# thu-nics/MixDQ

Hardware: AMD Instinct MI355X
Metric: sdxl_turbo_unet_w8a8_images_per_sec (higher is better)
Workload: dtype int8; 1 GPU; sdxl_turbo_unet_w8a8_1024px_bs1_1step; global_batch=1, per_gpu_batch=1, px=1024, latent=128, unet_forwards_per_image=1, unet_rows_per_image=1, graphs_cached=1, w_config=weight/uniform_8, a_config=act/act_8.00, bos=True, parallelism=dp1 (batch-sharded replicas, no step-loop collective), hip_graph=True, producer_fusions=True, swap_glue=False, w4_kernel_layers=0, quantizable_layers=794

## Files before the change

### __graft_entry__.py

```python
import os
import sys

ROOT = os.path.dirname(os.path.abspath(__file__))
if ROOT not in sys.path:
    sys.path.insert(0, ROOT)


def build() -> None:
    from mixdq_amd.build import build as build_hip
    lib = build_hip(force=False, verbose=True)
    assert os.path.exists(lib)
    from oracle import oracle as O
    O.build()
    import mixdq_amd._C as C
    import mixdq_amd.nn
    import mixdq_amd.quantize_sdxl
    import mixdq_amd.unet
    import mixdq_amd.text
    import mixdq_amd.image
    assert C.ABI_VERSION == 3
    print("build ok:", lib)


def smoke() -> None:
# ... 143 lines not shown
    xs, es = dd.f32(80, (2051,), -9, 9), dd.normal_f16(81, (2, 2056), 1.0)
    nz = dd.f32(82, (4, 2052), -2, 2)
    xs_d, in_d = t(xs), torch.zeros((2, 2056), dtype=torch.float16, device=dev)
    step_d, t_d = torch.tensor([1], dtype=torch.int32, device=dev), scal(-1.0)
    C.sampler_step(xs_d, t(es), in_d, t(sch.coef), t(sch.t_table), step_d, t_d, 7.5, 2, t(nz), n=2051, row_stride=2056,
                   noise_stride=2052)
    xs_ref, in_ref = sampler_ref.step(xs, es[0, :2051], es[1, :2051], sch.coef[1], 7.5, nz[1, :2051])
    assert np.array_equal(xs_d.cpu().numpy().view(np.uint32), xs_ref.view(np.uint32)), "sampler state mismatch"
    for r in range(2):
        assert np.array_equal(in_d[r, :2051].cpu().numpy().view(np.uint16), in_ref.view(np.uint16)), "sampler input"
    assert int(step_d.item()) == 2 and float(t_d.item()) == float(sch.timesteps[2]), "sampler step state"
    from tests import inpaint9_ref
    rng = np.random.default_rng(9)
    img = rng.integers(0, 256, (1, 3, 16, 24), dtype=np.uint8)
    msk = np.where(rng.random((1, 16, 24)) < 0.05, 255, 0).astype(np.uint8)
    grown = C.mask_dilate(t(msk), 2)
    assert np.array_equal(grown.cpu().numpy(), inpaint9_ref.mask_dilate(msk, 2)), "mask_dilate mismatch"
    blank = C.image_to_nhwc8_f16(t(img), grown).permute(0, 2, 3, 1).contiguous().cpu().numpy()
    assert np.array_equal(blank.view(np.uint16), inpaint9_ref.ingest_masked(img, grown.cpu().numpy()).view(np.uint16)), \
        "blanked ingest mismatch"
    ml, zl = dd.f32(90, (1, 2, 3), 0, 1), dd.f32(91, (1, 2, 3, 4), -3, 3)
    cnd = C.inpaint_cond(t(ml), t(zl).permute(0, 3, 1, 2)).permute(0, 2, 3, 1).contiguous().cpu().numpy()
    assert np.array_equal(cnd.view(np.uint16), inpaint9_ref.inpaint_cond(ml, zl).view(np.uint16)), "inpaint_cond mismatch"
    torch.cuda.synchronize()
    print("smoke ok: sampler step and the inpainting launches bit-exact vs their restatements; quantize, qlinear, qconv2d, qlinear_geglu, grouped GEMM, GroupNorm bit-exact vs oracle; "
          "fused cross-attention == its two-launch chain; the persistent GEMM + GEGLU kernel and a swapped "
          "GroupNorm + SiLU module bit-exact; attention and FP16 layers within tolerance "
          "on", torch.cuda.get_device_name(0))


if __name__ == "__main__":
    build()
    if "--smoke" in sys.argv:
        smoke()
```

### include/mixdq_hip.h

```cpp
#ifndef MIXDQ_HIP_H_
#define MIXDQ_HIP_H_

#include <stddef.h>
#include <stdint.h>

#ifdef __cplusplus
extern "C" {
#endif

#define MIXDQ_ABI_VERSION 3

typedef void* mixdq_stream_t;

enum mixdq_status {
  MIXDQ_OK = 0,
  MIXDQ_ERR_INVALID_ARG = 1,
  MIXDQ_ERR_ALIGNMENT = 2,
  MIXDQ_ERR_UNSUPPORTED = 3,
  MIXDQ_ERR_LAUNCH = 4,
  MIXDQ_ERR_W4_SHAPE = 5,
  MIXDQ_ERR_GEGLU_SHAPE = 6,
  MIXDQ_ERR_PADDING = 7,
  MIXDQ_ERR_ROWMAP_RESIDUAL = 8,
  MIXDQ_ERR_SHAPE = 9,
// ... 135 lines not shown
                         const float* scale_inv, const float* zero_point,
                         int8_t* out_q_or_null, void* out_f16_or_null, int flags,
                         mixdq_stream_t stream);

int mixdq_qlinear_w8a8_attn(const int8_t* A, const int8_t* W, const float* bias0, const float* scale,
                            const void* k_f16, const void* v_f16, void* out, int64_t M, int N, int K,
                            int rows_per_image, int tkv, int64_t k_batch_stride, int k_row_stride,
                            int64_t v_batch_stride, int v_row_stride, float softmax_scale,
                            const float* out_scale_inv_or_null, const float* out_zero_point_or_null,
                            int flags, mixdq_stream_t stream);

typedef struct mixdq_gemm_group {
  const int8_t* W;
  const float* bias0;
  const float* scale;
  const void* bias_f16_or_null;
  void* D_f16;
  int32_t N;
  int32_t reserved;
} mixdq_gemm_group;
int mixdq_qlinear_w8a8_grouped(const int8_t* A, const mixdq_gemm_group* groups_device, int ngroups,
                               int64_t M, int max_N, int K, int group_rows, int group_stride,
                               int group_offset, int flags, mixdq_stream_t stream);

int mixdq_qlinear_w8a8_geglu(const int8_t* A, const int8_t* W_interleaved, const float* bias0,
                             const float* scale, const void* bias_f16_or_null, int8_t* out_i8,
                             int64_t M, int N, int K, const float* out_scale_inv,
                             const float* out_zero_point, int flags, mixdq_stream_t stream);

int mixdq_attention_f16(const void* q_f16, const void* k_f16, const void* v_f16, void* out,
                        int batch, int heads, int head_dim, int tq, int tkv,
                        int64_t q_batch_stride, int64_t q_row_stride,
                        int64_t k_batch_stride, int64_t k_row_stride,
                        int64_t v_batch_stride, int64_t v_row_stride,
                        int64_t out_batch_stride, int64_t out_row_stride,
                        float softmax_scale, const float* out_scale_inv_or_null,
                        const float* out_zero_point_or_null, int flags, mixdq_stream_t stream);

int mixdq_attention_f16_prefetch(const void* q_f16, const void* k_f16, const void* v_f16, void* out,
                                 int batch, int heads, int head_dim, int tq, int tkv,
                                 int64_t q_batch_stride, int64_t q_row_stride,
                                 int64_t k_batch_stride, int64_t k_row_stride,
                                 int64_t v_batch_stride, int64_t v_row_stride,
                                 int64_t out_batch_stride, int64_t out_row_stride,
                                 float softmax_scale, const float* out_scale_inv_or_null,
                                 const float* out_zero_point_or_null,
// ... 119 lines not shown
```

### mixdq_amd/_C.py

```python
from __future__ import annotations

import ctypes
import os

import torch

_PKG = os.path.dirname(os.path.abspath(__file__))
LIB_PATH = os.environ.get("MIXDQ_HIP_LIB") or os.path.join(_PKG, "libmixdq_hip.so")

if not os.path.exists(LIB_PATH):
    raise ImportError(
        f"{LIB_PATH} not found: the HIP extension has not been built. Run "
        "`python -m mixdq_amd.build` (needs hipcc). There is no CPU fallback.")

_lib = ctypes.CDLL(LIB_PATH)

_vp, _i64, _i32, _sz = ctypes.c_void_p, ctypes.c_int64, ctypes.c_int, ctypes.c_size_t
_lib.mixdq_status_string.restype = ctypes.c_char_p
_lib.mixdq_status_string.argtypes = [_i32]
_lib.mixdq_abi_version.restype = _i32
_lib.mixdq_quantize_f16_i8.argtypes = [_vp, _vp, _vp, _vp, _vp, _i32, _vp, _vp, _i32, _vp]
_lib.mixdq_qlinear_w8a8.argtypes = [_vp, _vp, _vp, _vp, _vp, _vp, _i64, _i32, _i32, _i32, _vp]
_lib.mixdq_qlinear_w8a8_rows.argtypes = [_vp, _vp, _vp, _vp, _vp, _vp, _i64, _i32, _i32,
                                         _i32, _i32, _i32, _vp, _i64, _i32, _vp]
# ... 493 lines not shown
        _check(all(m[0].size(1) == self.members[0][0].size(1) for m in self.members),
               "members of a grouped launch share K")
        self.max_N = max(r[5] for r in rows)
        self.n = len(rows)
        self.table = torch.from_numpy(np.asarray(rows, dtype=np.int64)).to(self.members[0][0].device)
        self.key = tuple(r[0] for r in rows) + tuple(r[4] for r in rows)


def qlinear_grouped(input_int8, table: "GemmGroupTable", *, _row_map=None, _cfg=0):
    _check(input_int8.is_cuda and input_int8.dtype == torch.int8, "input_int8 should be int8 on GPU")
    _check(input_int8.size(-1) == table.K, "The last dimension of input and weight should match")
    a = input_int8.contiguous()
    M = a.numel() // table.K if table.K else 0
    rm = _row_map or (0, 0, 0)
    _record("linear_grouped", M, sum(m[0].size(0) for m in table.members), table.K, table.K,
            table.w4, qlinear_grouped,
            (input_int8, table), dict(_row_map=_row_map, _cfg=_cfg), w2=table.w2)
    with torch.cuda.device(a.device):
        code = _lib.mixdq_qlinear_w8a8_grouped(a.data_ptr(), table.table.data_ptr(), table.n, M,
                                               table.max_N, table.K, rm[0], rm[1], rm[2],
                                               FLAGS | (_cfg << 8) | _wflag(table.w4, table.w2),
                                               _stream())
    _status(code, "qlinear_grouped")


_lib.mixdq_qlinear_w8a8_attn.argtypes = [_vp] * 7 + [_i64, _i32, _i32, _i32, _i32, _i64, _i32, _i64,
                                          _i32, ctypes.c_float, _vp, _vp, _i32, _vp]
_lib.mixdq_qlinear_w8a8_attn.restype = _i32


def qlinear_attention_supported(x_shape, N, K, k) -> bool:
    return (len(x_shape) == 3 and N % 128 == 0 and K % 128 == 0 and x_shape[1] % 64 == 0
            and k.dim() == 3 and 0 < k.shape[1] <= 128 and k.shape[2] == N
            and x_shape[0] * x_shape[1] * K < 2 ** 32 and N * K < 2 ** 32)


def qlinear_attention(input_int8, weight_int8, scale, bias0, k, v, scale_inv=None, zero_point=None,
                      softmax_scale=None, *, _w4=False, _w2=False, _abits=8):
    _trace_w(weight_int8)
    _check(input_int8.is_cuda and input_int8.dtype == torch.int8 and input_int8.dim() == 3,
           "input_int8 should be an int8 [B, T, K] GPU tensor")
    _check(weight_int8.dtype == torch.int8, "weight_int8 should be int8 type")
    wflag = _wflag(_w4, _w2)
    N, K = weight_int8.size(0), weight_int8.size(1) * _kmul(_w4, _w2)
    B, T, _ = input_int8.shape
    _check(input_int8.size(-1) == K, "The last dimension of input and weight should match")
# ... 1005 lines not shown
```

### mixdq_amd/build.py

```python
import os
import subprocess
import sys

PKG = os.path.dirname(os.path.abspath(__file__))
CSRC = os.path.join(PKG, "csrc")
LIB = os.path.join(PKG, "libmixdq_hip.so")
SOURCES = ["quantize.hip", "igemm.hip", "igemm_aq.hip", "igemm_ln.hip", "iconv.hip", "fused_norm.hip", "attention.hip",
           "sampler.hip", "vae.hip", "image.hip"]
HEADERS = ["common.h", "attn_core.h", "iconv.h", "igemm_kernel.h", "igemm_pp.h", "f16in_table.h", os.path.join("..", "..", "include", "mixdq_hip.h"),
           os.path.join("..", "..", "include", "mixdq_math.h")]
FLAGS = ["--offload-arch=gfx950", "-O3", "-std=c++17", "-fPIC", "-ffp-contract=off",
         "-fno-fast-math", "-Wall", "-Wno-unused-function"]
EXTRA = {"attention.hip": ["-mllvm", "-amdgpu-mfma-vgpr-form=1"],
         "igemm.hip": ["-mllvm", "-amdgpu-kernarg-preload-count=14"],
         "igemm_aq.hip": ["-mllvm", "-amdgpu-kernarg-preload-count=14"],
         "igemm_ln.hip": ["-mllvm", "-amdgpu-kernarg-preload-count=14"]}
OBJ = os.path.join(PKG, "_obj")


def _hipcc():
    for c in (os.environ.get("HIPCC"), "/opt/rocm/bin/hipcc", "hipcc"):
        if c and (os.path.sep not in c or os.path.exists(c)):
            return c
    return "hipcc"


def csrc_sha16() -> str:
    import hashlib
    h = hashlib.sha256()
    for name in sorted(os.listdir(CSRC)):
        if name.endswith((".hip", ".h")):
            with open(os.path.join(CSRC, name), "rb") as f:
                h.update(name.encode() + b"\0" + f.read())
    return h.hexdigest()[:16]


def _build_info_obj(force: bool) -> str:
    src = os.path.join(OBJ, "build_info.cpp")
    obj = os.path.join(OBJ, "build_info.o")
    text = ('extern "C" __attribute__((visibility("default"))) const char* mixdq_build_csrc_sha16() '
            '{ return "%s"; }\n' % csrc_sha16())
    if force or not os.path.exists(src) or open(src).read() != text or not os.path.exists(obj):
        with open(src, "w") as f:
            f.write(text)
        subprocess.check_call(["g++", "-O1", "-fPIC", "-c", "-o", obj, src])
    return obj


def _aq_asm_cmd(asm: str):
    src = os.path.join(CSRC, "igemm_aq.hip")
    return [_hipcc()] + FLAGS + EXTRA.get("igemm_aq.hip", []) + ["--cuda-device-only", "-S", "-o", asm, src]


def _check_aq_isa(asm: str, obj: str) -> None:
    tool = os.path.join(os.path.dirname(PKG), "tools", "check_aq_isa.py")
    if not os.path.exists(tool):
# ... 53 lines not shown
```

### mixdq_amd/unet.py

```python
from __future__ import annotations

import math
import weakref
from collections import OrderedDict

import torch
import torch.nn as nn
import torch.nn.functional as F

DEFUSE = False


class defused:

    def __enter__(self):
        global DEFUSE
        self.saved, DEFUSE = DEFUSE, True

    def __exit__(self, *exc):
        global DEFUSE
        DEFUSE = self.saved


def _accel(m) -> bool:
# ... 286 lines not shown
    projection_class_embeddings_input_dim=None,
    use_linear_projection=False,
    norm_num_groups=32,
)

SDXL_INPAINT_CONFIG = dict(SDXL_CONFIG, in_channels=9)
SD15_INPAINT_CONFIG = dict(SD15_CONFIG, in_channels=9)


def head_width(cfg, channels: int) -> int:
    heads = cfg.get("num_attention_heads")
    if heads:
        if channels % heads:
            raise ValueError(f"{channels} channels do not split into {heads} heads")
        return channels // heads
    return cfg["head_dim"]


def _linear_proj(cfg) -> bool:
    return bool(cfg.get("use_linear_projection", True))


def sinusoidal_embedding(t: torch.Tensor, dim: int) -> torch.Tensor:
    half = dim // 2
    key = (half, t.device)
    freqs = _SIN_FREQS.get(key)
    if freqs is None:
        exponent = -math.log(10000.0) * torch.arange(half, dtype=torch.float32, device=t.device) / half
        freqs = torch.exp(exponent)
        if not (t.is_cuda and torch.cuda.is_current_stream_capturing()):
            _SIN_FREQS[key] = freqs
    emb = t.float()[:, None] * freqs[None, :]
    return torch.cat([torch.cos(emb), torch.sin(emb)], dim=-1)


_SIN_FREQS = {}


class TimestepEmbedding(nn.Module):
    def __init__(self, in_dim, dim):
        super().__init__()
        self.linear_1 = nn.Linear(in_dim, dim)
        self.linear_2 = nn.Linear(dim, dim)

    def forward(self, x):
        return self.linear_2(F.silu(self.linear_1(x)))


class ResnetBlock2D(nn.Module):
    def __init__(self, cin, cout, temb_dim, groups, split=0):
        super().__init__()
        self.norm1 = nn.GroupNorm(groups, cin, eps=1e-5)
        self.conv1 = nn.Conv2d(cin, cout, 3, 1, 1)
        self.time_emb_proj = nn.Linear(temb_dim, cout)
        self.norm2 = nn.GroupNorm(groups, cout, eps=1e-5)
        self.conv2 = nn.Conv2d(cout, cout, 3, 1, 1)
        self.conv_shortcut = nn.Conv2d(cin, cout, 1, 1, 0) if cin != cout else None
        self.nonlinearity = nn.SiLU()
        if self.conv_shortcut is not None and split:
# ... 646 lines not shown
            table = self._grouped("kv", (g, K, wb, B, T), [
                (pk["w"], pk["bias0"], pk["scale"], None, o) for _, pk, o in members], wb)
            _C.qlinear_grouped(x_int, table, _row_map=(T - 1, T, 1))

    @staticmethod
    def _kv_pack(blk, context=None):
        lk, lv = blk.attn2.to_k, blk.attn2.to_v
        layers = [lk, lv]
        if not (all(getattr(m, "valid_for_acceleration", False) and getattr(m, "bos", False)
                    and m.bias is None for m in layers)
                and lk.out_features == lv.out_features):
            return None
        if context is not None and not (context.dtype == torch.float16 and context.shape[1] > 1):
            return None
        if len(set(_quantizer_groups(_memo(blk), "kv", layers))) != 1:
            return None
        if not _uniform_storage(layers):
            return None
        pack = blk.__dict__.get("_kvpack")
        if not _pack_valid(pack, layers):
            pack = blk.__dict__["_kvpack"] = _pack_rows(layers)
        return pack

    def _project_temb_ahead(self, emb):
        resnets = [m for m in self.modules() if isinstance(m, ResnetBlock2D)]
        if not resnets or not emb.is_cuda:
            return
        s = F.silu(emb)
        B = s.shape[0]
        acc = [r.time_emb_proj for r in resnets if _accel(r.time_emb_proj)]
        ok = _fusable_f16(s) and s.dim() == 2
        gid = dict(zip(map(id, acc), _quantizer_groups(_memo(self), "temb", acc)))
        shared, grouped = {}, {}
        for res in resnets:
            layer = res.time_emb_proj
            if not (_accel(layer) and ok):
                res._t = (layer(s), None)
                continue
            bufs = layer.__dict__.setdefault("_t_out", {})
            buf = bufs.get((B, s.device))
            if buf is None:
                buf = bufs[(B, s.device)] = torch.empty((B, layer.out_features),
                                                        dtype=torch.float16, device=s.device)
            res._t = (buf, None)
            grouped.setdefault((gid[id(layer)], layer.in_features, _wbits(layer)),
                               []).append((layer, buf))
        from mixdq_amd import _C
        for (g, K, wb), members in grouped.items():
            if g not in shared:
                shared[g] = members[0][0]._quant(s)
            x_int = shared[g]
            if len(members) == 1:
                members[0][0]._gemm(x_int, out=members[0][1])
                continue
            table = self._grouped("temb", (g, K, wb, B), [
                (m.weight_storage()[0], m.bias0, m.scale, m.bias, buf)
                for m, buf in members], wb)
            _C.qlinear_grouped(x_int, table)

    def refresh_derived_(self):
        with torch.no_grad():
            for m in self.modules():
                if m is not self and hasattr(m, "refresh_derived_"):
                    m.refresh_derived_()
                bufs = m.__dict__.get("_kv_buf")
                if bufs and torch.is_tensor(getattr(m, "bos_pre_computed", None)):
                    for slot in bufs.values():
                        slot[1][:, :1, :] = m.bos_pre_computed.to(slot[1].device)
                        slot[0] = None
                pack = m.__dict__.get("_kvpack")
                if pack is not None and pack.get("outs"):
                    lk, lv = (r() for r in pack["layers"])
                    if lk is None or lv is None:
                        continue
                    for slot in pack["outs"].values():
                        slot[1][:, :1, :] = torch.cat(
                            [lk.bos_pre_computed, lv.bos_pre_computed], dim=-1).to(slot[1].device)
                        slot[0] = None
        return self

    def prepare_fused_(self):
# ... 110 lines not shown
                raise RuntimeError(f"SDXLUNet.forward: this UNet has {cc} conditioning channels: a {co}-channel sample "
                                   f"needs cond_term= (unet.cond_term(cond)), or pass all {co + cc} channels")
            return
        if cc <= 0:
            raise RuntimeError("SDXLUNet.forward: cond_term given, but this UNet has no conditioning channels")
        if sample.dim() != 4 or sample.shape[1] != co:
            raise RuntimeError(f"SDXLUNet.forward: with cond_term the sample should have {co} channels")
        want = (sample.shape[0], self.conv_in.out_channels, sample.shape[2], sample.shape[3])
        if not (torch.is_tensor(cond_term) and tuple(cond_term.shape) == want and cond_term.dtype == sample.dtype
                and cond_term.device == sample.device
                and cond_term.is_contiguous(memory_format=torch.channels_last)):
            raise RuntimeError(f"SDXLUNet.forward: cond_term should be a channels-last {sample.dtype} tensor of shape "
                               f"{want} (one row per sample row) on the sample's device")

    def forward(self, sample, timestep, encoder_hidden_states, added_cond_kwargs=None,
                return_dict=False, cond_term=None):
        cfg = self.cfg
        self._check_cond_term(sample, cond_term)
        B = sample.shape[0]
        dtype = sample.dtype
        t = timestep
        if not torch.is_tensor(t):
            t = torch.tensor([t], dtype=torch.float32, device=sample.device)
        t = t.reshape(-1).expand(B)
        emb = self.time_embedding(sinusoidal_embedding(t, cfg["block_out_channels"][0]).to(dtype))
        if cfg.get("addition_embed_type", "text_time") is not None:
            time_ids = added_cond_kwargs["time_ids"]
            text_embeds = added_cond_kwargs["text_embeds"]
            tid = sinusoidal_embedding(time_ids.flatten(), cfg["addition_time_embed_dim"])
            add = torch.cat([text_embeds, tid.reshape(B, -1).to(dtype)], dim=-1)
            emb = emb + self.add_embedding(add)

        use_pf = bool(self.fused and PREFETCH and sample.is_cuda and _fusable_f16(sample) and not DEFUSE)
        if not use_pf:
            return self._forward_body(sample, emb, encoder_hidden_states, cond_term)
        from mixdq_amd import _C
        plans = self.__dict__.setdefault("_pf_plans", {})
        plan = plans.get(sample.device)
        if plan is not None and not _plan_alive(plan, sample.device):
            plans.pop(sample.device, None)
            plan = None
        ctx = _C.PrefetchContext(sample.device, plan["lists"] if plan else None)
        try:
            with ctx:
                return self._forward_body(sample, emb, encoder_hidden_states, cond_term)
        finally:
            if ctx._outer is None:
                sig = _trace_signature(ctx.trace)
                if plan is None or plan["sig"] != sig:
                    new = _build_prefetch_plan(ctx.trace)
                    if new is None:
                        plans.pop(sample.device, None)
                    else:
                        plans[sample.device] = new

    def _apply(self, fn, recurse=True):
        self.__dict__.pop("_pf_plans", None)
        self.__dict__.pop("_cin_split", None)
        return super()._apply(fn, recurse)

    def load_state_dict(self, *args, **kwargs):
        self.__dict__.pop("_pf_plans", None)
        return super().load_state_dict(*args, **kwargs)

    def _forward_body(self, sample, emb, encoder_hidden_states, cond_term=None):
        if self.fused and _fusable_f16(sample) and not DEFUSE:
            self._project_temb_ahead(emb)
            self._project_context_ahead(encoder_hidden_states)
        x = sample.contiguous(memory_format=torch.channels_last)
        x = self.conv_in(x) if cond_term is None else self._conv_in_with_term(x, cond_term)
        skips = [x]
        for blk in self.down_blocks:
            x, outs = blk(x, emb, encoder_hidden_states)
            skips += outs
        x = self.mid_block(x, emb, encoder_hidden_states)
        for blk in self.up_blocks:
            x = blk(x, skips, emb, encoder_hidden_states)
        if self.fused and _fusable_f16(x):
            feed, q = _gn_feed(self.conv_norm_out, x, self.conv_out, silu=True)
            x = self.conv_out.forward_quantized(feed) if q else self.conv_out(feed)
        else:
            x = self.conv_out(self.conv_act(self.conv_norm_out(x)))
        return (x,)


def quantizable_layers(unet: nn.Module) -> "OrderedDict[str, nn.Module]":
    return OrderedDict((n, m) for n, m in unet.named_modules()
                       if isinstance(m, (nn.Linear, nn.Conv2d)))


# ... 19 lines not shown
```

Baseline: 92.19 images/s.

## Fuse conditioning embeddings into a cond prologue with grouped GEMV kernels

Adds a cond_embed kernel that builds the sinusoidal timestep and time-id embeddings and quantizes them directly. It also adds a grouped int8 GEMV kernel with SiLU+quantize and pair-add epilogues that computes the time/add embedding MLPs and writes the quantized temb inputs for the resnets. Together these replace the many small torch ops and GEMM launches at the start of the UNet forward. The path runs by default when batch is small, at the cost of a second code path and extra buffers.

Result: no change. 92.80 images/s (median of 6 runs) (+0.7%).

```diff
diff --git a/__graft_entry__.py b/__graft_entry__.py
--- a/__graft_entry__.py
+++ b/__graft_entry__.py
@@ -189,6 +189,16 @@
     ml, zl = dd.f32(90, (1, 2, 3), 0, 1), dd.f32(91, (1, 2, 3, 4), -3, 3)
     cnd = C.inpaint_cond(t(ml), t(zl).permute(0, 3, 1, 2)).permute(0, 2, 3, 1).contiguous().cpu().numpy()
     assert np.array_equal(cnd.view(np.uint16), inpaint9_ref.inpaint_cond(ml, zl).view(np.uint16)), "inpaint_cond mismatch"
+    gm, gw = [], []
+    for i, (n_out, k_in) in enumerate(((128, 320), (64, 192))):
+        xi, wi = dd.int8(95 + i, (2, k_in)), dd.int8(97 + i, (n_out, k_in))
+        b0i, sci = dd.f32(99 + i, (n_out,), -200, 200), dd.f32(101 + i, (n_out,), 2e-4, 9e-4)
+        oi = torch.zeros((2, n_out), dtype=torch.float16, device=dev)
+        gm.append((t(xi), t(wi), t(b0i), t(sci), None, oi, None, None, None))
+        gw.append(O.qlinear(xi, wi, b0i, sci, None, variant))
+    C.qlinear_gemv_grouped(C.GemvTable(gm))
+    for m_, want in zip(gm, gw):
+        assert np.array_equal(m_[5].cpu().numpy().view(np.uint16), want.view(np.uint16)), "GEMV mismatch"
     torch.cuda.synchronize()
     print("smoke ok: sampler step and the inpainting launches bit-exact vs their restatements; quantize, qlinear, qconv2d, qlinear_geglu, grouped GEMM, GroupNorm bit-exact vs oracle; "
           "fused cross-attention == its two-launch chain; the persistent GEMM + GEGLU kernel and a swapped "
diff --git a/include/mixdq_hip.h b/include/mixdq_hip.h
--- a/include/mixdq_hip.h
+++ b/include/mixdq_hip.h
@@ -181,6 +181,39 @@
 int mixdq_qlinear_w8a8_grouped(const int8_t* A, const mixdq_gemm_group* groups_device, int ngroups,
                                int64_t M, int max_N, int K, int group_rows, int group_stride,
                                int group_offset, int flags, mixdq_stream_t stream);
+
+typedef struct mixdq_gemv_group {
+  const int8_t* W;
+  const float* bias0;
+  const float* scale;
+  const void* bias_f16_or_null;
+  void* D_f16_or_null;
+  int32_t N;
+  int32_t K;
+  const int8_t* A;
+  int8_t* Q_or_null;
+  const float* q_scale_inv;
+  const float* q_zero_point;
+} mixdq_gemv_group;
+typedef struct mixdq_quant_out {
+  int8_t* out;
+  const float* scale_inv;
+  const float* zero_point;
+} mixdq_quant_out;
+enum { MIXDQ_GEMV_PLAIN = 0, MIXDQ_GEMV_SILU_QUANT = 1, MIXDQ_GEMV_PAIR_ADD_SILU_QUANT = 2 };
+#define MIXDQ_GEMV_MAX_PAIR_OUTS 8
+int mixdq_qlinear_w8a8_gemv_grouped(const mixdq_gemv_group* groups_device, const mixdq_gemv_group* groups_host,
+                                    int ngroups, int64_t M, int epilogue, const mixdq_quant_out* pair_outs,
+                                    int n_pair_outs, void* emb_f16_or_null, void* silu_f16_or_null, int flags,
+                                    mixdq_stream_t stream);
+int mixdq_qlinear_gemv_max_rows(void);
+
+enum { MIXDQ_COND_F32 = 0, MIXDQ_COND_F16 = 1, MIXDQ_COND_I64 = 2, MIXDQ_COND_I32 = 3, MIXDQ_COND_F64 = 4 };
+int mixdq_cond_embed(const void* timestep, int t_dtype, int t_count, const void* time_ids, int ids_dtype, int n_ids,
+                     const void* text_f16, int64_t text_row_stride, int P, const float* freqs0, int half0,
+                     const float* freqs1, int half1, void* out0, const float* scale_inv0, const float* zero_point0,
+                     void* out1, const float* scale_inv1, const float* zero_point1, int B, int flags,
+                     mixdq_stream_t stream);
 
 int mixdq_qlinear_w8a8_geglu(const int8_t* A, const int8_t* W_interleaved, const float* bias0,
                              const float* scale, const void* bias_f16_or_null, int8_t* out_i8,
diff --git a/mixdq_amd/_C.py b/mixdq_amd/_C.py
--- a/mixdq_amd/_C.py
+++ b/mixdq_amd/_C.py
@@ -539,6 +539,129 @@
                                                FLAGS | (_cfg << 8) | _wflag(table.w4, table.w2),
                                                _stream())
     _status(code, "qlinear_grouped")
+
+
+if not hasattr(_lib, "mixdq_qlinear_w8a8_gemv_grouped"):
+    raise ImportError(f"{LIB_PATH} does not export mixdq_qlinear_w8a8_gemv_grouped (rebuild with "
+                      "`python -m mixdq_amd.build --force`)")
+_lib.mixdq_qlinear_w8a8_gemv_grouped.argtypes = [_vp, _vp, _i32, _i64, _i32, _vp, _i32, _vp, _vp, _i32, _vp]
+_lib.mixdq_qlinear_w8a8_gemv_grouped.restype = _i32
+_lib.mixdq_qlinear_gemv_max_rows.argtypes = []
+_lib.mixdq_qlinear_gemv_max_rows.restype = _i32
+_lib.mixdq_cond_embed.argtypes = [_vp, _i32, _i32, _vp, _i32, _i32, _vp, _i64, _i32, _vp, _i32, _vp, _i32,
+                                  _vp, _vp, _vp, _vp, _vp, _vp, _i32, _i32, _vp]
+_lib.mixdq_cond_embed.restype = _i32
+
+GEMV_MAX_ROWS = int(_lib.mixdq_qlinear_gemv_max_rows())
+GEMV_MAX_PAIR_OUTS = 8
+GEMV_EPILOGUES = {None: 0, "silu_quant": 1, "pair": 2}
+COND_DTYPES = {torch.float32: 0, torch.float16: 1, torch.int64: 2, torch.int32: 3, torch.float64: 4}
+
+
+def cond_prologue_enabled() -> bool:
+    return os.environ.get("MIXDQ_COND_PROLOGUE", "1") != "0"
+
+
+def gemv_wanted(M: int) -> bool:
+    return 0 < int(M) <= GEMV_MAX_ROWS
+
+
+class GemvTable:
+
+    def __init__(self, members):
+        import numpy as np
+        rows, keep = [], []
+        self.M = None
+        for a, w, b0, sc, bias, out, q_out, q_sinv, q_zp in members:
+            _check(w.is_cuda and w.dtype == torch.int8 and w.dim() == 2 and w.is_contiguous(), "member weight: int8 [N, K]")
+            N, K = w.shape
+            _check(a.is_cuda and a.dtype == torch.int8 and a.is_contiguous() and a.dim() >= 1 and a.shape[-1] == K,
+                   "member input: contiguous int8 [..., K]")
+            M = a.numel() // K if K else 0
+            _check(self.M in (None, M), "members of a GEMV launch have the same number of rows")
+            self.M = M
+            b0, sc = _f32vec(b0), _f32vec(sc)
+            bias = None if bias is None else bias.contiguous()
+            _check(b0.numel() == N and sc.numel() == N and (bias is None or (bias.numel() == N and bias.dtype == torch.float16)),
+                   "member epilogue vectors should have N elements (bias: fp16)")
+            for t, dt, n in ((out, torch.float16, "out"), (q_out, torch.int8, "q_out")):
+                _check(t is None or (t.is_cuda and t.dtype == dt and t.is_contiguous() and t.numel() == M * N),
+                       f"member {n}: contiguous [M, N]")
+            _check((q_out is None) == (q_sinv is None) == (q_zp is None), "q_out comes with its quantizer")
+            _check(q_sinv is None or (q_sinv.dtype == torch.float32 and q_zp.dtype == torch.float32),
+                   "quantizer parameters should be fp32")
+            keep.append((a, w, b0, sc, bias, out, q_out, q_sinv, q_zp))
+            rows.append([w.data_ptr(), b0.data_ptr(), sc.data_ptr(), _ptr(bias) or 0, _ptr(out) or 0,
+                         int(N) | (int(K) << 32), a.data_ptr(), _ptr(q_out) or 0, _ptr(q_sinv) or 0, _ptr(q_zp) or 0])
+        self._keep = keep
+        self.n = len(rows)
+        self.shapes = tuple((r[5] & 0xffffffff, r[5] >> 32) for r in rows)
+        self.host = np.ascontiguousarray(np.asarray(rows, dtype=np.int64).reshape(self.n, 10))
+        self.table = torch.from_numpy(self.host).to(keep[0][0].device) if rows else None
+        self.key = tuple(v for r in rows for v in r)
+
+
+def qlinear_gemv_grouped(table: "GemvTable", *, _epilogue=None, _pair_outs=(), _emb=None, _silu=None):
+    import numpy as np
+    _check(_epilogue in GEMV_EPILOGUES, f"_epilogue: one of {list(GEMV_EPILOGUES)}")
+    if table.n == 0 or not table.M:
+        return
+    dev = table.table.device
+    po = None
+    if _epilogue == "pair":
+        _check(len(_pair_outs) <= GEMV_MAX_PAIR_OUTS, f"at most {GEMV_MAX_PAIR_OUTS} pair outputs")
+        N = table.shapes[0][0]
+        for q, s, z in _pair_outs:
+            _check(q.is_cuda and q.dtype == torch.int8 and q.is_contiguous() and q.numel() == table.M * N
+                   and s.dtype == torch.float32 and z.dtype == torch.float32 and s.device == dev and z.device == dev,
+                   "pair output: contiguous int8 [M, N] with fp32 quantizer parameters")
+        for t in (_emb, _silu):
+            _check(t is None or (t.is_cuda and t.dtype == torch.float16 and t.is_contiguous()
+                                 and t.numel() == table.M * N), "emb / silu: contiguous fp16 [M, N]")
+        po = np.ascontiguousarray(np.asarray([[q.data_ptr(), s.data_ptr(), z.data_ptr()] for q, s, z in _pair_outs],
+                                             dtype=np.int64).reshape(len(_pair_outs), 3))
+    else:
+        _check(not _pair_outs and _emb is None and _silu is None, "pair outputs belong to the pair epilogue")
+    _record("linear_gemv", table.M, sum(s[0] for s in table.shapes), max(s[1] for s in table.shapes),
+            min(s[1] for s in table.shapes), False, qlinear_gemv_grouped, (table,),
+            dict(_epilogue=_epilogue, _pair_outs=_pair_outs, _emb=_emb, _silu=_silu))
+    with torch.cuda.device(dev):
+        code = _lib.mixdq_qlinear_w8a8_gemv_grouped(
+            table.table.data_ptr(), table.host.ctypes.data, table.n, table.M, GEMV_EPILOGUES[_epilogue],
+            None if po is None or not len(po) else po.ctypes.data, 0 if po is None else len(po), _ptr(_emb), _ptr(_silu),
+            FLAGS, _stream())
+    _status(code, "qlinear_gemv_grouped")
+
+
+def cond_embed(timestep, time_ids, text_embeds, freqs0, freqs1, q0=None, q1=None, *, _out0=None, _out1=None):
+    dev = text_embeds.device
+    _check(text_embeds.is_cuda and text_embeds.dtype == torch.float16 and text_embeds.dim() == 2
+           and (text_embeds.shape[1] == 0 or text_embeds.stride(1) == 1), "text_embeds should be fp16 [B, P] on GPU")
+    B, P = text_embeds.shape
+    _check(timestep.device == dev and timestep.dtype in COND_DTYPES and timestep.numel() in (1, B)
+           and timestep.is_contiguous(), "timestep: 1 or B values on the device")
+    _check(time_ids.device == dev and time_ids.dtype in COND_DTYPES and time_ids.dim() == 2 and time_ids.shape[0] == B
+           and time_ids.is_contiguous(), "time_ids: contiguous [B, n] on the device")
+    for f in (freqs0, freqs1):
+        _check(f.device == dev and f.dtype == torch.float32 and f.dim() == 1 and f.is_contiguous(), "freqs: fp32 vector")
+    for q in (q0, q1):
+        _check(q is None or all(t.device == dev and t.dtype == torch.float32 for t in q), "quantizer parameters: fp32")
+    h0, h1, n = freqs0.numel(), freqs1.numel(), time_ids.shape[1]
+    outs = []
+    for given, q, width in ((_out0, q0, 2 * h0), (_out1, q1, P + n * 2 * h1)):
+        dt = torch.float16 if q is None else torch.int8
+        _check(given is None or (given.device == dev and given.dtype == dt and given.shape == (B, width)
+                                 and given.is_contiguous()), "_out<i>: a contiguous [B, width] buffer of the output's type")
+        outs.append(torch.empty((B, width), dtype=dt, device=dev) if given is None else given)
+    out0, out1 = outs
+    with torch.cuda.device(dev):
+        code = _lib.mixdq_cond_embed(
+            timestep.data_ptr(), COND_DTYPES[timestep.dtype], timestep.numel(), time_ids.data_ptr(),
+            COND_DTYPES[time_ids.dtype], n, text_embeds.data_ptr(), text_embeds.stride(0) if B > 1 else P, P,
+            freqs0.data_ptr(), h0, freqs1.data_ptr(), h1, out0.data_ptr(), _ptr(q0 and q0[0]), _ptr(q0 and q0[1]),
+            out1.data_ptr(), _ptr(q1 and q1[0]), _ptr(q1 and q1[1]), B, FLAGS, _stream())
+    _status(code, "cond_embed")
+    return out0, out1
 
 
 _lib.mixdq_qlinear_w8a8_attn.argtypes = [_vp] * 7 + [_i64, _i32, _i32, _i32, _i32, _i64, _i32, _i64,
diff --git a/mixdq_amd/build.py b/mixdq_amd/build.py
--- a/mixdq_amd/build.py
+++ b/mixdq_amd/build.py
@@ -4,9 +4,10 @@
 
 PKG = os.path.dirname(os.path.abspath(__file__))
 CSRC = os.path.join(PKG, "csrc")
+INCLUDE = os.path.join(os.path.dirname(PKG), "include")
 LIB = os.path.join(PKG, "libmixdq_hip.so")
 SOURCES = ["quantize.hip", "igemm.hip", "igemm_aq.hip", "igemm_ln.hip", "iconv.hip", "fused_norm.hip", "attention.hip",
-           "sampler.hip", "vae.hip", "image.hip"]
+           "sampler.hip", "vae.hip", "image.hip", "cond.hip"]
 HEADERS = ["common.h", "attn_core.h", "iconv.h", "igemm_kernel.h", "igemm_pp.h", "f16in_table.h", os.path.join("..", "..", "include", "mixdq_hip.h"),
            os.path.join("..", "..", "include", "mixdq_math.h")]
 FLAGS = ["--offload-arch=gfx950", "-O3", "-std=c++17", "-fPIC", "-ffp-contract=off",
@@ -32,6 +33,10 @@
         if name.endswith((".hip", ".h")):
             with open(os.path.join(CSRC, name), "rb") as f:
                 h.update(name.encode() + b"\0" + f.read())
+    for name in sorted(os.listdir(INCLUDE)):
+        if name.endswith(".h"):
+            with open(os.path.join(INCLUDE, name), "rb") as f:
+                h.update(b"include/" + name.encode() + b"\0" + f.read())
     return h.hexdigest()[:16]
 
 
diff --git a/mixdq_amd/csrc/cond.hip b/mixdq_amd/csrc/cond.hip
--- /dev/null
+++ b/mixdq_amd/csrc/cond.hip
@@ -0,0 +1,340 @@
+#include "common.h"
+
+namespace mixdq {
+namespace {
+
+__device__ __forceinline__ float load_as_float(const void* p, int dtype, int64_t i) {
+  switch (dtype) {
+    case MIXDQ_COND_F16: return __half2float(reinterpret_cast<const __half*>(p)[i]);
+    case MIXDQ_COND_I64: return (float)reinterpret_cast<const int64_t*>(p)[i];
+    case MIXDQ_COND_I32: return (float)reinterpret_cast<const int32_t*>(p)[i];
+    case MIXDQ_COND_F64: return (float)reinterpret_cast<const double*>(p)[i];
+    default: return reinterpret_cast<const float*>(p)[i];
+  }
+}
+
+__device__ __forceinline__ __half silu_f16(__half h) {
+  const float x = __half2float(h);
+  const float e = expf(-x);
+  return f32_to_f16_rn(x / __fadd_rn(1.0f, e));
+}
+
+__device__ __forceinline__ int8_t quantize_f16(__half h, float s_inv, float zp, bool unfused) {
+  const float x = __half2float(h);
+  return (int8_t)(unfused ? quantize_one<true>(x, s_inv, zp) : quantize_one<false>(x, s_inv, zp));
+}
+
+struct EmbedArgs {
+  const void* t; const void* ids; const __half* text;
+  const float* f0; const float* f1;
+  void* out0; void* out1;
+  const float* s0; const float* z0; const float* s1; const float* z1;
+  int64_t text_stride;
+  int t_dtype, t_n, ids_dtype, n_ids, P, half0, half1, B, unfused;
+};
+
+__global__ __launch_bounds__(256) void cond_embed_kernel(EmbedArgs a) {
+  const int w0 = 2 * a.half0, w1 = a.P + a.n_ids * 2 * a.half1;
+  const int64_t e = (int64_t)blockIdx.x * blockDim.x + threadIdx.x;
+  if (e >= (int64_t)a.B * (w0 + w1)) return;
+  const int b = (int)(e / (w0 + w1));
+  int c = (int)(e - (int64_t)b * (w0 + w1));
+  const bool second = c >= w0;
+  __half h;
+  if (second && c - w0 < a.P) {
+    c -= w0;
+    h = a.text[b * a.text_stride + c];
+  } else {
+    float v;
+    const float* f;
+    int half, i;
+    if (!second) {
+      v = load_as_float(a.t, a.t_dtype, a.t_n > 1 ? b : 0);
+      f = a.f0; half = a.half0; i = c;
+    } else {
+      c -= w0;
+      const int r = c - a.P;
+      v = load_as_float(a.ids, a.ids_dtype, (int64_t)b * a.n_ids + r / (2 * a.half1));
+      f = a.f1; half = a.half1; i = r % (2 * a.half1);
+    }
+    const bool is_sin = i >= half;
+    const float arg = __fmul_rn(v, f[is_sin ? i - half : i]);
+    h = f32_to_f16_rn(is_sin ? sinf(arg) : cosf(arg));
+  }
+  void* out = second ? a.out1 : a.out0;
+  const float* sp = second ? a.s1 : a.s0;
+  const float* zp = second ? a.z1 : a.z0;
+  const int64_t o = (int64_t)b * (second ? w1 : w0) + c;
+  if (sp) reinterpret_cast<int8_t*>(out)[o] = quantize_f16(h, *sp, *zp, a.unfused != 0);
+  else reinterpret_cast<__half*>(out)[o] = h;
+}
+
+constexpr int kGemvMaxRows = 8;
+constexpr int kGemvWaves = 4;
+constexpr int kGemvTargetWaves = 4096;
+constexpr int kGemvMaxLds = 64 * 1024;
+
+__host__ __device__ inline int gemv_lanes(int K) {
+  const int chunks = K >> 4;
+  int l = 4;
+  while (l < 64 && l * 4 < chunks) l <<= 1;
+  return l;
+}
+
+struct PairOuts {
+  mixdq_quant_out q[MIXDQ_GEMV_MAX_PAIR_OUTS];
+  int n;
+  __half* emb; __half* silu;
+};
+
+template <int MR>
+__device__ __forceinline__ void gemv_dot(const mixdq_gemv_group& g, const char* a_lds, int col, bool valid, int kl,
+                                         int lanes, int (&acc)[MR]) {
+  const int chunks = g.K >> 4;
+  const uint4* wrow = reinterpret_cast<const uint4*>(g.W + (int64_t)col * g.K);
+#pragma unroll
+  for (int m = 0; m < MR; ++m) acc[m] = 0;
+  for (int j0 = kl; j0 < chunks; j0 += 4 * lanes) {
+    uint4 w[4];
+#pragma unroll
+    for (int u = 0; u < 4; ++u) {
+      const int j = j0 + u * lanes;
+      w[u] = (valid && j < chunks) ? wrow[j] : make_uint4(0, 0, 0, 0);
+    }
+#pragma unroll
+    for (int u = 0; u < 4; ++u) {
+      const int j = min(j0 + u * lanes, chunks - 1);
+#pragma unroll
+      for (int m = 0; m < MR; ++m) {
+        const uint4 av = *reinterpret_cast<const uint4*>(a_lds + m * g.K + j * 16);
+        int s = acc[m];
+        s = __builtin_amdgcn_sdot4((int)av.x, (int)w[u].x, s, false);
+        s = __builtin_amdgcn_sdot4((int)av.y, (int)w[u].y, s, false);
+        s = __builtin_amdgcn_sdot4((int)av.z, (int)w[u].z, s, false);
+        s = __builtin_amdgcn_sdot4((int)av.w, (int)w[u].w, s, false);
+        acc[m] = s;
+      }
+    }
+  }
+}
+
+template <int MR, int EPI>
+__global__ __launch_bounds__(256) void gemv_kernel(const mixdq_gemv_group* __restrict__ groups, int M, int ppt,
+                                                   int unfused_, PairOuts po) {
+  extern __shared__ __attribute__((aligned(16))) char gemv_lds[];
+  constexpr int NM = EPI == 2 ? 2 : 1;
+  mixdq_gemv_group g[NM];
+#pragma unroll
+  for (int h = 0; h < NM; ++h) g[h] = groups[blockIdx.y * NM + h];
+  const int N = g[0].N;
+  int lanes = gemv_lanes(g[0].K);
+  if (NM == 2) lanes = max(lanes, gemv_lanes(g[NM - 1].K));
+  const int cpp = 64 / lanes;
+  const int cw = ppt * cpp;
+  const int block_col0 = blockIdx.x * (kGemvWaves * cw);
+  if (block_col0 >= N) return;
+  const bool unfused = unfused_ != 0;
+
+  int a_off[NM];
+  {
+    int off = 0;
+#pragma unroll
+    for (int h = 0; h < NM; ++h) {
+      a_off[h] = off;
+      const int chunks = g[h].K >> 4;
+      const uint4* src = reinterpret_cast<const uint4*>(g[h].A);
+      uint4* dst = reinterpret_cast<uint4*>(gemv_lds + off);
+      for (int i = threadIdx.x; i < MR * chunks; i += blockDim.x)
+        dst[i] = i < M * chunks ? src[i] : make_uint4(0, 0, 0, 0);
+      off += MR * g[h].K;
+    }
+  }
+  float q_sinv = 0.f, q_zp = 0.f;
+  if constexpr (EPI == 1) { q_sinv = *g[0].q_scale_inv; q_zp = *g[0].q_zero_point; }
+  float p_sinv[MIXDQ_GEMV_MAX_PAIR_OUTS], p_zp[MIXDQ_GEMV_MAX_PAIR_OUTS];
+  if constexpr (EPI == 2) {
+#pragma unroll
+    for (int i = 0; i < MIXDQ_GEMV_MAX_PAIR_OUTS; ++i)
+      if (i < po.n) { p_sinv[i] = *po.q[i].scale_inv; p_zp[i] = *po.q[i].zero_point; }
+  }
+  __syncthreads();
+
+  const int lane = threadIdx.x & 63, wave = threadIdx.x >> 6;
+  const int kl = lane & (lanes - 1), sub = lane / lanes;
+  const int wave_col0 = block_col0 + wave * cw;
+  for (int p = 0; p < ppt; ++p) {
+    const int c0 = wave_col0 + p * cpp;
+    if (c0 >= N) break;
+    const int col = c0 + sub;
+    const bool valid = col < N;
+    const int colc = valid ? col : N - 1;
+    float b0[NM], sc[NM], bs[NM];
+#pragma unroll
+    for (int h = 0; h < NM; ++h) {
+      b0[h] = g[h].bias0[colc];
+      sc[h] = g[h].scale[colc];
+      bs[h] = g[h].bias_f16_or_null ? __half2float(reinterpret_cast<const __half*>(g[h].bias_f16_or_null)[colc]) : 0.f;
+    }
+    int acc[NM][MR];
+#pragma unroll
+    for (int h = 0; h < NM; ++h) gemv_dot<MR>(g[h], gemv_lds + a_off[h], colc, valid, kl, lanes, acc[h]);
+#pragma unroll
+    for (int o = 32; o >= 1; o >>= 1) {
+      if (o < lanes) {
+#pragma unroll
+        for (int h = 0; h < NM; ++h)
+#pragma unroll
+          for (int m = 0; m < MR; ++m) acc[h][m] += __shfl_xor(acc[h][m], o);
+      }
+    }
+#pragma unroll
+    for (int m = 0; m < MR; ++m) {
+      if (kl != 0 || !valid || m >= M) break;
+      const int64_t o = (int64_t)m * N + col;
+      __half d[NM];
+#pragma unroll
+      for (int h = 0; h < NM; ++h) {
+        d[h] = epilogue_one(acc[h][m], b0[h], sc[h], bs[h], g[h].bias_f16_or_null != nullptr, unfused);
+        if (g[h].D_f16_or_null) reinterpret_cast<__half*>(g[h].D_f16_or_null)[o] = d[h];
+      }
+      if constexpr (EPI == 1) {
+        g[0].Q_or_null[o] = quantize_f16(silu_f16(d[0]), q_sinv, q_zp, unfused);
+      } else if constexpr (EPI == 2) {
+        const __half emb = f32_to_f16_rn(__fadd_rn(__half2float(d[0]), __half2float(d[NM - 1])));
+        const __half s = silu_f16(emb);
+        if (po.emb) po.emb[o] = emb;
+        if (po.silu) po.silu[o] = s;
+#pragma unroll
+        for (int i = 0; i < MIXDQ_GEMV_MAX_PAIR_OUTS; ++i)
+          if (i < po.n) po.q[i].out[o] = quantize_f16(s, p_sinv[i], p_zp[i], unfused);
+      }
+    }
+  }
+}
+
+template <int EPI>
+int launch_gemv(const mixdq_gemv_group* dev, int M, int ppt, int unfused, const PairOuts& po, dim3 grid, int lds,
+                hipStream_t stream) {
+#define GEMV_GO(MR) gemv_kernel<MR, EPI><<<grid, 64 * kGemvWaves, lds, stream>>>(dev, M, ppt, unfused, po)
+  if (M == 1) GEMV_GO(1);
+  else if (M == 2) GEMV_GO(2);
+  else if (M <= 4) GEMV_GO(4);
+  else GEMV_GO(8);
+#undef GEMV_GO
+  return launch_status();
+}
+
+inline bool dtype_ok(int d) { return d >= MIXDQ_COND_F32 && d <= MIXDQ_COND_F64; }
+inline int dtype_size(int d) { return d == MIXDQ_COND_F16 ? 2 : (d == MIXDQ_COND_F32 || d == MIXDQ_COND_I32) ? 4 : 8; }
+
+}
+}
+
+using namespace mixdq;
+
+extern "C" int mixdq_qlinear_gemv_max_rows(void) { return kGemvMaxRows; }
+
+extern "C" int mixdq_cond_embed(const void* timestep, int t_dtype, int t_count, const void* time_ids, int ids_dtype,
+                                int n_ids, const void* text_f16, int64_t text_row_stride, int P, const float* freqs0,
+                                int half0, const float* freqs1, int half1, void* out0, const float* scale_inv0,
+                                const float* zero_point0, void* out1, const float* scale_inv1,
+                                const float* zero_point1, int B, int flags, mixdq_stream_t stream) {
+  if (flags & ~MIXDQ_FLAG_UNFUSED) return MIXDQ_ERR_UNSUPPORTED;
+  if (B < 0 || P < 0 || n_ids < 0 || half0 < 0 || half1 < 0 || text_row_stride < 0) return MIXDQ_ERR_INVALID_ARG;
+  if (!dtype_ok(t_dtype) || !dtype_ok(ids_dtype) || (t_count != 1 && t_count != B)) return MIXDQ_ERR_INVALID_ARG;
+  if ((scale_inv0 == nullptr) != (zero_point0 == nullptr) || (scale_inv1 == nullptr) != (zero_point1 == nullptr))
+    return MIXDQ_ERR_INVALID_ARG;
+  const int64_t w0 = 2 * (int64_t)half0, w1 = (int64_t)P + (int64_t)n_ids * 2 * half1;
+  if (w0 + w1 > INT32_MAX) return MIXDQ_ERR_SHAPE;
+  const int64_t total = (int64_t)B * (w0 + w1);
+  if (total == 0) return MIXDQ_OK;
+  if ((w0 && (!timestep || !freqs0 || !out0)) || (w1 && !out1) || (P && !text_f16) ||
+      (n_ids * half1 && (!time_ids || !freqs1)))
+    return MIXDQ_ERR_INVALID_ARG;
+  if (((uintptr_t)timestep % dtype_size(t_dtype)) || ((uintptr_t)time_ids % dtype_size(ids_dtype)) ||
+      ((uintptr_t)text_f16 & 1) || (((uintptr_t)freqs0 | (uintptr_t)freqs1) & 3) ||
+      (!scale_inv0 && ((uintptr_t)out0 & 1)) || (!scale_inv1 && ((uintptr_t)out1 & 1)))
+    return MIXDQ_ERR_ALIGNMENT;
+  EmbedArgs a;
+  a.t = timestep; a.ids = time_ids; a.text = (const __half*)text_f16;
+  a.f0 = freqs0; a.f1 = freqs1; a.out0 = out0; a.out1 = out1;
+  a.s0 = scale_inv0; a.z0 = zero_point0; a.s1 = scale_inv1; a.z1 = zero_point1;
+  a.text_stride = text_row_stride;
+  a.t_dtype = t_dtype; a.t_n = t_count; a.ids_dtype = ids_dtype; a.n_ids = n_ids; a.P = P;
+  a.half0 = half0; a.half1 = half1; a.B = B; a.unfused = (flags & MIXDQ_FLAG_UNFUSED) ? 1 : 0;
+  const int64_t blocks = (total + 255) / 256;
+  if (blocks > INT32_MAX) return MIXDQ_ERR_SHAPE;
+  cond_embed_kernel<<<(int)blocks, 256, 0, (hipStream_t)stream>>>(a);
+  return launch_status();
+}
+
+extern "C" int mixdq_qlinear_w8a8_gemv_grouped(const mixdq_gemv_group* groups_device,
+                                               const mixdq_gemv_group* groups_host, int ngroups, int64_t M,
+                                               int epilogue, const mixdq_quant_out* pair_outs, int n_pair_outs,
+                                               void* emb_f16_or_null, void* silu_f16_or_null, int flags,
+                                               mixdq_stream_t stream) {
+  if (flags & ~MIXDQ_FLAG_UNFUSED) return MIXDQ_ERR_UNSUPPORTED;
+  if (M < 0 || ngroups < 0 || n_pair_outs < 0) return MIXDQ_ERR_INVALID_ARG;
+  if (epilogue < MIXDQ_GEMV_PLAIN || epilogue > MIXDQ_GEMV_PAIR_ADD_SILU_QUANT) return MIXDQ_ERR_INVALID_ARG;
+  if (M == 0 || ngroups == 0) return MIXDQ_OK;
+  if (M > kGemvMaxRows) return MIXDQ_ERR_SHAPE;
+  if (!groups_device || !groups_host || ngroups > 65535) return MIXDQ_ERR_INVALID_ARG;
+  const bool pair = epilogue == MIXDQ_GEMV_PAIR_ADD_SILU_QUANT;
+  const int nm = pair ? 2 : 1;
+  PairOuts po{};
+  if (pair) {
+    if (ngroups != 2 || n_pair_outs > MIXDQ_GEMV_MAX_PAIR_OUTS || (n_pair_outs && !pair_outs))
+      return MIXDQ_ERR_INVALID_ARG;
+    if (groups_host[0].N != groups_host[1].N) return MIXDQ_ERR_SHAPE;
+    for (int i = 0; i < n_pair_outs; ++i) {
+      if (!pair_outs[i].out || !pair_outs[i].scale_inv || !pair_outs[i].zero_point) return MIXDQ_ERR_INVALID_ARG;
+      po.q[i] = pair_outs[i];
+    }
+    po.n = n_pair_outs;
+    po.emb = (__half*)emb_f16_or_null;
+    po.silu = (__half*)silu_f16_or_null;
+    if (((uintptr_t)po.emb | (uintptr_t)po.silu) & 1) return MIXDQ_ERR_ALIGNMENT;
+  } else if (n_pair_outs || emb_f16_or_null || silu_f16_or_null) {
+    return MIXDQ_ERR_INVALID_ARG;
+  }
+  const int mr = M == 1 ? 1 : M == 2 ? 2 : M <= 4 ? 4 : 8;
+  int64_t passes = 0;
+  int lds = 0;
+  for (int i = 0; i < ngroups; i += nm) {
+    int lanes = 0, lds_i = 0;
+    for (int h = 0; h < nm; ++h) {
+      const mixdq_gemv_group& g = groups_host[i + h];
+      if (!g.W || !g.bias0 || !g.scale || !g.A || g.N <= 0 || g.K <= 0) return MIXDQ_ERR_INVALID_ARG;
+      if (g.N % 4 != 0 || g.K % 16 != 0 || (((uintptr_t)g.W | (uintptr_t)g.A) & 15) ||
+          (((uintptr_t)g.bias0 | (uintptr_t)g.scale) & 3) ||
+          (((uintptr_t)g.bias_f16_or_null | (uintptr_t)g.D_f16_or_null) & 1))
+        return MIXDQ_ERR_ALIGNMENT;
+      if (epilogue == MIXDQ_GEMV_SILU_QUANT && (!g.Q_or_null || !g.q_scale_inv || !g.q_zero_point))
+        return MIXDQ_ERR_INVALID_ARG;
+      if (epilogue == MIXDQ_GEMV_PLAIN && !g.D_f16_or_null) return MIXDQ_ERR_INVALID_ARG;
+      lanes = lanes > gemv_lanes(g.K) ? lanes : gemv_lanes(g.K);
+      lds_i += mr * g.K;
+    }
+    if (lds_i > kGemvMaxLds) return MIXDQ_ERR_SHAPE;
+    lds = lds > lds_i ? lds : lds_i;
+    const int cpp = 64 / lanes;
+    passes += (groups_host[i].N + cpp - 1) / cpp;
+  }
+  int64_t ppt = passes / kGemvTargetWaves;
+  if (ppt < 1) ppt = 1;
+  if (ppt > 1024) ppt = 1024;
+  int gx = 1;
+  for (int i = 0; i < ngroups; i += nm) {
+    int lanes = 0;
+    for (int h = 0; h < nm; ++h) lanes = lanes > gemv_lanes(groups_host[i + h].K) ? lanes : gemv_lanes(groups_host[i + h].K);
+    const int64_t cols_per_block = (int64_t)kGemvWaves * ppt * (64 / lanes);
+    const int64_t bx = (groups_host[i].N + cols_per_block - 1) / cols_per_block;
+    gx = gx > bx ? gx : (int)bx;
+  }
+  const dim3 grid(gx, ngroups / nm, 1);
+  const int unfused = (flags & MIXDQ_FLAG_UNFUSED) ? 1 : 0;
+  hipStream_t s = (hipStream_t)stream;
+  if (epilogue == MIXDQ_GEMV_PLAIN) return launch_gemv<0>(groups_device, (int)M, (int)ppt, unfused, po, grid, lds, s);
+  if (epilogue == MIXDQ_GEMV_SILU_QUANT) return launch_gemv<1>(groups_device, (int)M, (int)ppt, unfused, po, grid, lds, s);
+  return launch_gemv<2>(groups_device, (int)M, (int)ppt, unfused, po, grid, lds, s);
+}
diff --git a/mixdq_amd/unet.py b/mixdq_amd/unet.py
--- a/mixdq_amd/unet.py
+++ b/mixdq_amd/unet.py
@@ -332,19 +332,41 @@
 
 
 def sinusoidal_embedding(t: torch.Tensor, dim: int) -> torch.Tensor:
-    half = dim // 2
-    key = (half, t.device)
-    freqs = _SIN_FREQS.get(key)
-    if freqs is None:
-        exponent = -math.log(10000.0) * torch.arange(half, dtype=torch.float32, device=t.device) / half
-        freqs = torch.exp(exponent)
-        if not (t.is_cuda and torch.cuda.is_current_stream_capturing()):
-            _SIN_FREQS[key] = freqs
+    freqs = _sin_freqs(dim // 2, t.device)
     emb = t.float()[:, None] * freqs[None, :]
     return torch.cat([torch.cos(emb), torch.sin(emb)], dim=-1)
 
 
+def _sin_freqs(half: int, device, cached_only: bool = False):
+    key = (half, torch.device(device))
+    freqs = _SIN_FREQS.get(key)
+    if freqs is None and not cached_only:
+        exponent = -math.log(10000.0) * torch.arange(half, dtype=torch.float32, device=device) / half
+        freqs = torch.exp(exponent)
+        if not (freqs.is_cuda and torch.cuda.is_current_stream_capturing()):
+            _SIN_FREQS[key] = freqs
+    return freqs
+
+
 _SIN_FREQS = {}
+
+
+def cond_layers_reason(layers):
+    for m in layers:
+        if not _accel(m):
+            return "an embedding layer is not an accelerated W8A8 layer"
+        if _wbits(m) != 8:
+            return "an embedding layer stores packed 4- or 2-bit weights"
+        if not _a8(m):
+            return "an embedding layer has a 4-bit activation quantizer"
+        if m.in_features % 16 != 0 or m.out_features % 4 != 0:
+            return "an embedding layer's sizes are outside the GEMV's (K % 16, N % 4)"
+    return None
+
+
+def temb_route(rows: int, wbits: int) -> str:
+    from mixdq_amd import _C
+    return "gemv" if _C.cond_prologue_enabled() and _C.gemv_wanted(rows) and wbits == 8 else "grouped"
 
 
 class TimestepEmbedding(nn.Module):
@@ -1037,34 +1059,45 @@
             pack = blk.__dict__["_kvpack"] = _pack_rows(layers)
         return pack
 
-    def _project_temb_ahead(self, emb):
+    def _project_temb_ahead(self, emb, pre=None):
         resnets = [m for m in self.modules() if isinstance(m, ResnetBlock2D)]
-        if not resnets or not emb.is_cuda:
+        if not resnets or not (pre is not None or emb.is_cuda):
             return
-        s = F.silu(emb)
-        B = s.shape[0]
+        from mixdq_amd import _C
         acc = [r.time_emb_proj for r in resnets if _accel(r.time_emb_proj)]
-        ok = _fusable_f16(s) and s.dim() == 2
         gid = dict(zip(map(id, acc), _quantizer_groups(_memo(self), "temb", acc)))
-        shared, grouped = {}, {}
+        if pre is None:
+            s = F.silu(emb)
+            shared = {}
+            ok = _fusable_f16(s) and s.dim() == 2
+        else:
+            s, shared = pre
+            ok = True
+        like = next(iter(shared.values())) if shared else s
+        B, dev = like.shape[0], like.device
+        grouped = {}
         for res in resnets:
             layer = res.time_emb_proj
             if not (_accel(layer) and ok):
                 res._t = (layer(s), None)
                 continue
             bufs = layer.__dict__.setdefault("_t_out", {})
-            buf = bufs.get((B, s.device))
+            buf = bufs.get((B, dev))
             if buf is None:
-                buf = bufs[(B, s.device)] = torch.empty((B, layer.out_features),
-                                                        dtype=torch.float16, device=s.device)
+                buf = bufs[(B, dev)] = torch.empty((B, layer.out_features),
+                                                   dtype=torch.float16, device=dev)
             res._t = (buf, None)
             grouped.setdefault((gid[id(layer)], layer.in_features, _wbits(layer)),
                                []).append((layer, buf))
-        from mixdq_amd import _C
+        gemv = []
         for (g, K, wb), members in grouped.items():
             if g not in shared:
                 shared[g] = members[0][0]._quant(s)
             x_int = shared[g]
+            if pre is not None and temb_route(B, wb) == "gemv":
+                gemv += [(x_int, m.weight_storage()[0], m.bias0, m.scale, m.bias, buf, None, None, None)
+                         for m, buf in members]
+                continue
             if len(members) == 1:
                 members[0][0]._gemm(x_int, out=members[0][1])
                 continue
@@ -1072,6 +1105,107 @@
                 (m.weight_storage()[0], m.bias0, m.scale, m.bias, buf)
                 for m, buf in members], wb)
             _C.qlinear_grouped(x_int, table)
+        if gemv:
+            _C.qlinear_gemv_grouped(self._gemv_table("temb", (B, dev), gemv))
+
+    def _gemv_table(self, name, key, members):
+        from mixdq_amd._C import GemvTable
+        tables = self.__dict__.setdefault("_gemv_tables", {})
+        want = tuple(0 if t is None else t.data_ptr() for m in members for t in m)
+        t = tables.get((name, key))
+        if t is None or t.src_key != want:
+            t = tables[(name, key)] = GemvTable(members)
+            t.src_key = want
+        return t
+
+    def _cond_prologue_reason(self, sample, timestep, added_cond_kwargs):
+        from mixdq_amd import _C
+        if not _C.cond_prologue_enabled():
+            return "MIXDQ_COND_PROLOGUE=0"
+        if not self.fused or DEFUSE:
+            return "not the fused graph"
+        if not _fusable_f16(sample):
+            return "sample is not FP16 on the GPU"
+        B, dev = sample.shape[0], sample.device
+        if not _C.gemv_wanted(B):
+            return f"batch {B}: more rows than the GEMV takes"
+        if getattr(self, "add_embedding", None) is None or not isinstance(added_cond_kwargs, dict):
+            return "no addition embedding"
+        ids, text = added_cond_kwargs.get("time_ids"), added_cond_kwargs.get("text_embeds")
+        if not (torch.is_tensor(ids) and torch.is_tensor(text) and torch.is_tensor(timestep)):
+            return "conditioning inputs are not tensors"
+        if not (text.device == dev and text.dtype == torch.float16 and text.dim() == 2 and text.shape[0] == B
+                and text.stride(1) == 1):
+            return "text_embeds is not FP16 [B, P] on the sample's device"
+        if not (ids.device == dev and ids.dtype in _C.COND_DTYPES and ids.dim() == 2 and ids.shape[0] == B
+                and ids.is_contiguous()):
+            return "time_ids is not a contiguous [B, n] tensor on the sample's device"
+        if not (timestep.device == dev and timestep.dtype in _C.COND_DTYPES and timestep.numel() in (1, B)
+                and timestep.is_contiguous()):
+            return "timestep is not 1 or B values on the sample's device"
+        te, ae = self.time_embedding, self.add_embedding
+        why = cond_layers_reason((te.linear_1, te.linear_2, ae.linear_1, ae.linear_2))
+        if why:
+            return why
+        cfg = self.cfg
+        h0, h1 = cfg["block_out_channels"][0] // 2, cfg["addition_time_embed_dim"] // 2
+        if te.linear_1.in_features != 2 * h0 or ae.linear_1.in_features != text.shape[1] + ids.shape[1] * 2 * h1:
+            return "embedding widths do not match the layers"
+        if ae.linear_2.out_features != te.linear_2.out_features:
+            return "the two embeddings differ in width"
+        capturing = torch.cuda.is_current_stream_capturing()
+        if any(_sin_freqs(h, dev, cached_only=capturing) is None for h in (h0, h1)):
+            return "frequency tables not built yet (never inside a capture)"
+        acc = [m.time_emb_proj for m in self.modules() if isinstance(m, ResnetBlock2D) and _accel(m.time_emb_proj)]
+        if any(not _a8(m) for m in acc):
+            return "a time_emb_proj layer has a 4-bit activation quantizer"
+        if acc and (capturing and _memo(self).get("temb") is None):
+            return "quantizer grouping not taken yet (never inside a capture)"
+        if len(set(_quantizer_groups(_memo(self), "temb", acc))) > _C.GEMV_MAX_PAIR_OUTS:
+            return "more time_emb_proj quantizer groups than the pair epilogue writes"
+        return None
+
+    def _cond_prologue(self, sample, timestep, added_cond_kwargs):
+        from mixdq_amd import _C
+        cfg = self.cfg
+        te, ae = self.time_embedding, self.add_embedding
+        ids, text = added_cond_kwargs["time_ids"], added_cond_kwargs["text_embeds"]
+        B, dev = sample.shape[0], sample.device
+        f0 = _sin_freqs(cfg["block_out_channels"][0] // 2, dev)
+        f1 = _sin_freqs(cfg["addition_time_embed_dim"] // 2, dev)
+        resnets = [m for m in self.modules() if isinstance(m, ResnetBlock2D)]
+        acc = [r.time_emb_proj for r in resnets if _accel(r.time_emb_proj)]
+        gids = _quantizer_groups(_memo(self), "temb", acc)
+        first = {}
+        for g, m in zip(gids, acc):
+            first.setdefault(g, m)
+        need_f16 = len(acc) != len(resnets) or not all(r.fused for r in resnets)
+        T = te.linear_2.out_features
+        bufs = self.__dict__.setdefault("_cond_bufs", {})
+        b = bufs.get((B, dev))
+        if b is None:
+            i8 = lambda n: torch.empty((B, n), dtype=torch.int8, device=dev)
+            b = bufs[(B, dev)] = dict(x0=i8(te.linear_1.in_features), x1=i8(ae.linear_1.in_features),
+                                      h0=i8(te.linear_1.out_features), h1=i8(ae.linear_1.out_features), q={},
+                                      emb=torch.empty((B, T), dtype=torch.float16, device=dev),
+                                      silu=torch.empty((B, T), dtype=torch.float16, device=dev))
+        for g in first:
+            if g not in b["q"]:
+                b["q"][g] = torch.empty((B, T), dtype=torch.int8, device=dev)
+        _C.cond_embed(timestep, ids, text, f0, f1, _qp(te.linear_1), _qp(ae.linear_1), _out0=b["x0"], _out1=b["x1"])
+        def lin(x, m, q, nxt):
+            return (x, m.weight_int, m.bias0, m.scale, m.bias, None, q,
+                    None if nxt is None else nxt.act_scales_inv, None if nxt is None else nxt.act_zero_points)
+        _C.qlinear_gemv_grouped(self._gemv_table("cond1", (B, dev), [
+            lin(b["x0"], te.linear_1, b["h0"], te.linear_2), lin(b["x1"], ae.linear_1, b["h1"], ae.linear_2)]),
+            _epilogue="silu_quant")
+        outs = [(b["q"][g], m.act_scales_inv, m.act_zero_points) for g, m in first.items()]
+        _C.qlinear_gemv_grouped(self._gemv_table("cond2", (B, dev), [
+            lin(b["h0"], te.linear_2, None, None), lin(b["h1"], ae.linear_2, None, None)]),
+            _epilogue="pair", _pair_outs=outs, _emb=b["emb"] if need_f16 else None,
+            _silu=b["silu"] if need_f16 else None)
+        self._project_temb_ahead(None, pre=(b["silu"] if need_f16 else None, {g: b["q"][g] for g in first}))
+        return b["emb"] if need_f16 else None
 
     def refresh_derived_(self):
         with torch.no_grad():
@@ -1228,6 +1362,10 @@
         t = timestep
         if not torch.is_tensor(t):
             t = torch.tensor([t], dtype=torch.float32, device=sample.device)
+        ahead = self._cond_prologue_reason(sample, t.reshape(-1), added_cond_kwargs) is None
+        if ahead:
+            emb = self._cond_prologue(sample, t.reshape(-1), added_cond_kwargs)
+            return self._forward_from_emb(sample, emb, encoder_hidden_states, cond_term, True)
         t = t.reshape(-1).expand(B)
         emb = self.time_embedding(sinusoidal_embedding(t, cfg["block_out_channels"][0]).to(dtype))
         if cfg.get("addition_embed_type", "text_time") is not None:
@@ -1236,10 +1374,12 @@
             tid = sinusoidal_embedding(time_ids.flatten(), cfg["addition_time_embed_dim"])
             add = torch.cat([text_embeds, tid.reshape(B, -1).to(dtype)], dim=-1)
             emb = emb + self.add_embedding(add)
-
+        return self._forward_from_emb(sample, emb, encoder_hidden_states, cond_term, False)
+
+    def _forward_from_emb(self, sample, emb, encoder_hidden_states, cond_term, temb_ahead):
         use_pf = bool(self.fused and PREFETCH and sample.is_cuda and _fusable_f16(sample) and not DEFUSE)
         if not use_pf:
-            return self._forward_body(sample, emb, encoder_hidden_states, cond_term)
+            return self._forward_body(sample, emb, encoder_hidden_states, cond_term, temb_ahead)
         from mixdq_amd import _C
         plans = self.__dict__.setdefault("_pf_plans", {})
         plan = plans.get(sample.device)
@@ -1249,7 +1389,7 @@
         ctx = _C.PrefetchContext(sample.device, plan["lists"] if plan else None)
         try:
             with ctx:
-                return self._forward_body(sample, emb, encoder_hidden_states, cond_term)
+                return self._forward_body(sample, emb, encoder_hidden_states, cond_term, temb_ahead)
         finally:
             if ctx._outer is None:
                 sig = _trace_signature(ctx.trace)
@@ -1269,9 +1409,10 @@
         self.__dict__.pop("_pf_plans", None)
         return super().load_state_dict(*args, **kwargs)
 
-    def _forward_body(self, sample, emb, encoder_hidden_states, cond_term=None):
+    def _forward_body(self, sample, emb, encoder_hidden_states, cond_term=None, temb_ahead=False):
         if self.fused and _fusable_f16(sample) and not DEFUSE:
-            self._project_temb_ahead(emb)
+            if not temb_ahead:
+                self._project_temb_ahead(emb)
             self._project_context_ahead(encoder_hidden_states)
         x = sample.contiguous(memory_format=torch.channels_last)
         x = self.conv_in(x) if cond_term is None else self._conv_in_with_term(x, cond_term)
```
